# linomp/INF560-approximate-pattern-matching

Hardware: AMD Instinct MI355X
Metric: window-DP-cells/sec (higher is better)
Workload: dtype u32

## Files before the change

### inf560-approximate-pattern-matching_amd/csrc/apm_runtime.hip

```cpp
#include "apm_runtime.h"
#include "apm_core.h"

#include <cstdarg>
#include <cstdio>
#include <cstring>
#include <mutex>
#include <string>
#include <thread>
#include <vector>

static thread_local std::string g_create_error;

int fail(apm_ctx *ctx, int code, const char *fmt, ...) {
    char buf[512];
    va_list ap;
    va_start(ap, fmt);
    vsnprintf(buf, sizeof buf, fmt, ap);
    va_end(ap);
    static std::mutex mu;
    std::lock_guard<std::mutex> lock(mu);
    if (ctx) ctx->err = buf;
    else g_create_error = buf;
    return code;
}
// ... 236 lines not shown
            return fail(nullptr, APM_ERR_NO_DEVICE, "%d devices requested, APM_DEVICES lists %d", n_devices, (int)devs.size());
        return create_common(ctx, devs, true);
    }
    if (n_devices <= 0) n_devices = have;
    if (n_devices > have) return fail(nullptr, APM_ERR_NO_DEVICE, "%d devices requested, %d visible", n_devices, have);
    if (n_devices > apm_ctx::N_STAGE / 2) return fail(nullptr, APM_ERR_NO_DEVICE, "at most %d devices per context", apm_ctx::N_STAGE / 2);
    for (int i = 0; i < n_devices; ++i) devs.push_back(i);
    return create_common(ctx, devs, true);
}

int apm_create_on_device(apm_ctx **ctx, int device_id) {
    if (!ctx) return fail(nullptr, APM_ERR_INVALID, "ctx is NULL");
    *ctx = nullptr;
    const int have = apm_device_count();
    if (have < 0) return have;
    if (have == 0) return fail(nullptr, APM_ERR_NO_DEVICE, "no HIP device visible (this engine has no CPU fallback)");
    if (device_id < 0 || device_id >= have)
        return fail(nullptr, APM_ERR_NO_DEVICE, "device %d out of range (%d visible)", device_id, have);
    return create_common(ctx, std::vector<int>{device_id}, false);
}

void apm_destroy(apm_ctx *ctx) {
    if (!ctx) return;
    for (apm_ctx *ch : ctx->children) apm_destroy(ch);
    ctx->children.clear();
    if (ctx->rccl.ready)
        for (void *c : ctx->rccl.comms) if (c) ctx->rccl.CommDestroy(c);
    for (auto &ds : ctx->devs) {
        if (ds.dev < 0) continue;
        hipSetDevice(ds.dev);
        if (ds.own_stream) hipStreamSynchronize(ds.own_stream);
        free_device_plan(ds);
        for (void *p : {(void *)ds.d_scratch, (void *)ds.d_text, (void *)ds.d_rec, (void *)ds.d_rec_n, (void *)ds.d_ops, (void *)ds.d_masks, (void *)ds.d_stats,
                        (void *)ds.d_work, (void *)ds.d_blist, (void *)ds.d_clist, (void *)ds.d_clist_cnt, (void *)ds.d_raw, (void *)ds.d_tn_summary,
                        (void *)ds.d_tn_map, (void *)ds.d_tn_total, (void *)ds.d_sq_count, (void *)ds.d_sq_prefix, (void *)ds.d_sq_total,
                        (void *)ds.d_seq_table, (void *)ds.d_loc_buf, (void *)ds.d_best})
            if (p) hipFree(p);
        for (hipEvent_t e : ds.ev_best) if (e) hipEventDestroy(e);
        for (hipEvent_t e : ds.ev_stage) if (e) hipEventDestroy(e);
        for (hipEvent_t e : ds.ev_launch) if (e) hipEventDestroy(e);
        for (hipEvent_t e : ds.ev_tn) if (e) hipEventDestroy(e);
        for (hipEvent_t e : ds.ev_sq) if (e) hipEventDestroy(e);
        for (hipEvent_t e : {ds.ev_start, ds.ev_kstart, ds.ev_mstart, ds.ev_mstop, ds.ev_stop}) if (e) hipEventDestroy(e);
        if (ds.own_stream) hipStreamDestroy(ds.own_stream);
    }
    for (int b = 0; b < apm_ctx::N_STAGE; ++b)
        if (ctx->stage[b]) hipHostFree(ctx->stage[b]);
    delete ctx;
}

int apm_set_stream(apm_ctx *ctx, void *hip_stream) {
    if (!ctx) return APM_ERR_INVALID;
    if (ctx->devs.size() != 1) return fail(ctx, APM_ERR_STATE, "apm_set_stream needs a single-device context");
    ctx->devs[0].stream = hip_stream == APM_STREAM_OWN ? ctx->devs[0].own_stream : (hipStream_t)hip_stream;
    return APM_OK;
}

int apm_set_partition(apm_ctx *ctx, int partition) {
    if (!ctx) return APM_ERR_INVALID;
    if (partition != APM_PARTITION_TEXT && partition != APM_PARTITION_PATTERNS) return fail(ctx, APM_ERR_INVALID, "unknown partition %d", partition);
    if (partition == ctx->partition) return APM_OK;
    ctx->partition = partition;
    return ctx->pats.empty() ? (int)APM_OK : rebuild(ctx);
}

int apm_set_patterns(apm_ctx *ctx, int n_patterns, const char *const *pat, const int *len, int k) {
    if (!ctx) return APM_ERR_INVALID;
// ... 130 lines not shown
```

### inf560-approximate-pattern-matching_amd/csrc/apm_scan.hip

```cpp
#include "apm_state.h"
#include "apm_core.h"

#include <algorithm>
#include <cstdlib>
#include <cstring>

__global__ void apm_popcount_kernel(const uint32_t *w, unsigned long long n, unsigned long long *sum) {
    unsigned long long acc = 0;
    for (unsigned long long i = (unsigned long long)blockIdx.x * blockDim.x + threadIdx.x; i < n; i += (unsigned long long)gridDim.x * blockDim.x)
        acc += (unsigned long long)__popc(w[i]);
    for (int d = 32; d; d >>= 1) acc += __shfl_down(acc, d, 64);
    if ((threadIdx.x & 63) == 0 && acc) atomicAdd(sum, acc);
}

__global__ void apm_popcount_listed_kernel(const uint32_t *w, const uint32_t *blist, const uint32_t *n_listed, const uint32_t *clist_cnt, int regions, unsigned long long *sum) {
    unsigned long long acc = 0;
    const unsigned long long n = (unsigned long long)*n_listed * 64ull, t0 = (unsigned long long)blockIdx.x * blockDim.x + threadIdx.x;
    for (unsigned long long i = t0; i < n; i += (unsigned long long)gridDim.x * blockDim.x)
        acc += (unsigned long long)__popc(w[(unsigned long long)blist[i >> 6] * 64ull + (i & 63ull)]);
    for (unsigned long long i = t0; i < (unsigned long long)regions; i += (unsigned long long)gridDim.x * blockDim.x) acc += clist_cnt[i];
    for (int d = 32; d; d >>= 1) acc += __shfl_down(acc, d, 64);
    if ((threadIdx.x & 63) == 0 && acc) atomicAdd(sum, acc);
}

// ... 15 lines not shown
        const unsigned long long i = b0 + threadIdx.x, at = s_base + threadIdx.x;
        if (i < total && at < cap) {
            const unsigned long long pos = ob + i % span;
            out[at] = make_uint4((uint32_t)pos, (uint32_t)(pos >> 32), (uint32_t)idx[i / span], 0u);
        }
    }
}

int note_launch(apm_ctx *ctx, DeviceState &ds, const char *label) {
    ds.launches++;
    if (!ctx->timing_on || ds.n_stamps >= DeviceState::MAX_STAMPS) return APM_OK;
    hipEvent_t &e = ds.ev_launch[ds.n_stamps];
    if (!e) HIP_TRY(ctx, hipEventCreate(&e));
    HIP_TRY(ctx, hipEventRecord(e, ds.stream));
    ds.launch_label[ds.n_stamps++] = label;
    return APM_OK;
}

int ensure_text(apm_ctx *ctx, DeviceState &ds, size_t bytes) {
    bytes = (bytes + 255) & ~(size_t)255;
    if (bytes <= ds.text_cap) return APM_OK;
    HIP_TRY(ctx, hipSetDevice(ds.dev));
    return grow_device_buffer(ctx, ds, (void **)&ds.d_text, &ds.text_cap, bytes, 1);
}

static int env_int(const char *name, int unset) { const char *v = getenv(name); return v ? atoi(v) : unset; }
static int env_1_to_64(const char *name, int unset) { return getenv(name) ? std::max(1, std::min(64, env_int(name, 0))) : unset; }
struct ScanEnv {
    int fused = env_int("APM_FUSED", -1);
    int blist = env_int("APM_SIEVE_BLIST", 1);
    int clist = env_int("APM_SIEVE_CLIST", 1);
    int clist_region_cap = env_1_to_64("APM_CLIST_REGION_CAP", 0);
    int clist_min_batch = env_1_to_64("APM_CLIST_MIN_BATCH", 8);
    int cf_dp_diag = env_int("APM_CF_DP_DIAG", 1);
    int filter_dma = env_int("APM_FILTER_DMA", 1);
    int filter_stream = env_int("APM_FILTER_STREAM", 1);
#ifdef APM_MEASURE
    int qcap_s1 = env_int("APM_QCAP_S1", 0);
    int bpc_cap = env_int("APM_BPC_CAP", 0);
#endif
};
static const ScanEnv &scan_env() {
    static const ScanEnv env;
    return env;
}

struct ShardGeom {
    const uint8_t *text;
    int64_t jb, je;
    int64_t nrel;
    int64_t avail;
    int64_t avail_pad;
    int band;
    ApmPosSink sink;
    unsigned long long *counts;
    bool rec_on;
    bool aligned() const { return (reinterpret_cast<uintptr_t>(text) & 15u) == 0; }
};
#define APM_PICK(g, fn) ((g).rec_on ? fn##_rec : fn)

template <typename Args> static void set_common(Args &a, const apm_ctx *ctx, const ShardGeom &g, int64_t je) {
    a.text = g.text;
    a.jb = g.jb;
    a.je = je;
    a.nrel = g.nrel;
    a.counts = g.counts;
// ... 24 lines not shown
static int launch_generic_group(apm_ctx *ctx, DeviceState &ds, const ShardGeom &g, const GenericGroup &grp, const ApmPatDesc *d_descs, int mode) {
    if (grp.descs.empty() || g.je <= g.jb) return APM_OK;
    int64_t span = g.je - g.jb;
    if (mode == 1) span = std::min<int64_t>(span, grp.m_max);
    const size_t col = (size_t)grp.m_max + 1;
    const size_t budget = (size_t)1 << 30;
    const size_t per_launch = std::min<size_t>(grp.descs.size(), 65535);
    int64_t nbx = (span + APM_BLOCK - 1) / APM_BLOCK;
    const int64_t cap = std::max<int64_t>(1, (int64_t)(budget / (col * 2 * APM_BLOCK * per_launch)));
    nbx = std::max<int64_t>(1, std::min<int64_t>(std::min<int64_t>(nbx, cap), 4096));
    const size_t need = col * 2 * APM_BLOCK * (size_t)nbx * per_launch;
    const int rc = grow_device_buffer(ctx, ds, (void **)&ds.d_scratch, &ds.scratch_bytes, need, 1);
    if (rc) return rc;
    ApmGenericArgs a{};
    set_common(a, ctx, g, g.je);
    a.avail = g.avail;
    a.bytes = ds.d_allpat;
    a.mode = mode;
    a.col_stride = (int)col;
    a.scratch = ds.d_scratch;
    for (size_t first = 0; first < grp.descs.size(); first += per_launch) {
        a.pats = d_descs + first;
        APM_LAUNCH(ctx, ds, "generic", APM_PICK(g, apm_launch_generic)(a, (int)nbx, (int)std::min(per_launch, grp.descs.size() - first), ds.stream));
    }
    return APM_OK;
}

struct SieveRange {
    int64_t p_lo, p_hi;
    int64_t n_mask_blocks = 0;
    const uint32_t *blist_ctr = nullptr;
    int clist_regions = 0;
    uint32_t clist_region_cap = 0;
    int64_t nchunks() const { return (p_hi - p_lo + 1023) / 1024; }
};
constexpr int kClistPerBlock = 32;
constexpr int kClistMaxRegions = 4096;

static ApmSieve2Args sieve_args(const SievePlan &S, const ShardGeom &g, const SieveRange &r, const uint32_t *d_bitmap) {
    ApmSieve2Args sv{};
    sv.text = g.text;
    sv.avail_pad = g.avail_pad;
    sv.tile0 = r.p_lo;
    sv.nchunks = r.nchunks();
    sv.bitmap = reinterpret_cast<const uint4 *>(d_bitmap);
    sv.code_shift = S.code_shift;
    sv.stride = S.stride;
    return sv;
}

static ApmVerifyArgs verify_args(const apm_ctx *ctx, const VerifyLaunch &V, const DevVerify &D, const ShardGeom &g, int64_t je_v) {
    const SievePlan &S = ctx->plan.sieve;
    ApmVerifyArgs va{};
    set_common(va, ctx, g, je_v);
    va.avail = g.avail;
    va.avail_pad = g.avail_pad;
    va.image = reinterpret_cast<const uint4 *>(D.d_image);
    va.image_len = (int)V.image.size();
    va.o_prefix = V.o_prefix;
    va.o_r2s = V.o_r2s;
    va.o_slots = V.o_slots;
    va.o_kext = V.o_kext;
    va.o_pat = V.o_pat;
    va.o_masks = V.o_masks;
    va.o_kinfo = V.o_kinfo;
    va.o_pinfo = V.o_pinfo;
// ... 18 lines not shown
    for (size_t v = 0; fused_ok && v < S.launches.size(); ++v) {
        const VerifyLaunch &V = S.launches[v];
        DevVerify &D = ds.verify[v];
        ApmFusedArgs fa{};
        fa.s = sieve_args(S, g, r, ds.d_sieve_bmp);
        fa.v = verify_args(ctx, V, D, g, std::min<int64_t>(g.je, g.nrel - V.m_min + 1));
#ifdef APM_MEASURE
        if (!ds.d_stats) HIP_TRY(ctx, hipMalloc((void **)&ds.d_stats, APM_STATS_BYTES));
        fa.v.stats = ds.d_stats;
#endif
        if (!D.fused_threads) {
            D.fused_blocks_per_cu = apm_fused_geometry(fa, &D.fused_threads);
            if (D.fused_blocks_per_cu < 1) D.fused_threads = -1;
        }
        if (D.fused_threads < 64) fused_ok = false;
        if (fa.v.je > g.jb) { fargs.push_back(fa); fa_index.push_back(v); }
    }
    if (!fused_ok) return APM_OK;
    for (ApmFusedArgs &fa : fargs) {
        tails.ride_with(fa.s);
        const DevVerify &D = ds.verify[fa_index[&fa - fargs.data()]];
#ifdef APM_MEASURE
        HIP_TRY(ctx, hipMemsetAsync(ds.d_stats, 0, APM_STATS_BYTES, ds.stream));
#endif
        fa.v.work = ds.d_work;
        APM_LAUNCH(ctx, ds, "fused", APM_PICK(g, apm_launch_fused)(fa, D.fused_threads, ds.n_cu * D.fused_blocks_per_cu, &ds.work_epoch, ds.stream));
    }
    *ran = true;
    return APM_OK;
}

static int sieve_pass(apm_ctx *ctx, DeviceState &ds, const ShardGeom &g, SieveRange &r, ShortTails &tails, int v) {
    const SievePlan &S = ctx->plan.sieve;
    ApmSieve2Args sv = sieve_args(S, g, r, v < 0 ? ds.d_sieve_bmp : ds.verify[(size_t)v].d_bmp18);
    sv.masks = ds.d_masks;
    if (v >= 0) {
        const VerifyLaunch &V = S.launches[(size_t)v];
        const DevVerify &D = ds.verify[(size_t)v];
        sv.cf_image = reinterpret_cast<const uint4 *>(D.d_cf);
        sv.cf_len = (int)V.cf_image.size();
        sv.cf_o_rrec = V.cf_o_rrec;
        sv.cf_o_lrec = V.cf_o_lrec;
        sv.cf_threads = D.cf_threads;
        sv.cf_blocks_per_cu = D.cf_blocks_per_cu;
        sv.cf_o_dp = V.cf_o_dp;
        sv.cf_dp_k = ctx->k;
        sv.cf_dp_cols = V.cf_dp_cols;
    }
    if (v < 0 || tails.n <= 512) tails.ride_with(sv);
    const bool use_blist = scan_env().blist && sv.cf_image != nullptr;
    r.blist_ctr = nullptr;
    if (use_blist) {
        sv.blist = ds.d_blist;
        sv.blist_ctr = APM_BLIST_CTR(ds.d_work, ds.sieve_epoch & 1);
        sv.blist_ctr_next = APM_BLIST_CTR(ds.d_work, (ds.sieve_epoch + 1) & 1);
        r.blist_ctr = sv.blist_ctr;
    }
    r.clist_regions = 0;
    if (use_blist && scan_env().clist) {
        const size_t want = (size_t)r.n_mask_blocks * (size_t)kClistPerBlock + (size_t)kClistMaxRegions * 64;
        const int grc = grow_device_buffer(ctx, ds, (void **)&ds.d_clist, &ds.clist_cap, want, 4);
        if (grc) return grc;
        if (!ds.d_clist_cnt) HIP_TRY(ctx, hipMalloc((void **)&ds.d_clist_cnt, (size_t)kClistMaxRegions * 4));
        const int regions = apm_sieve2cf_blocks(sv, ds.n_cu);
        if (regions >= 1 && regions <= kClistMaxRegions) {
            r.clist_regions = regions;
            r.clist_region_cap = scan_env().clist_region_cap ? (uint32_t)scan_env().clist_region_cap
                                                             : (uint32_t)std::max<int64_t>(64, r.n_mask_blocks * kClistPerBlock / regions);
            sv.clist = ds.d_clist;
            sv.clist_cnt = ds.d_clist_cnt;
            sv.clist_cap = r.clist_region_cap;
        }
    }
    ds.last_clist_regions = r.clist_regions;
    ds.last_blist_ctr = r.blist_ctr;
    HIP_TRY(ctx, APM_PICK(g, apm_launch_sieve2)(sv, ds.n_cu, ds.stream, scan_env().cf_dp_diag != 0, &ds.last_sieve_waves, &ds.last_cf_dp_form));
    if (use_blist) ++ds.sieve_epoch;
    return note_launch(ctx, ds, "sieve");
}

static int verify_pass(apm_ctx *ctx, DeviceState &ds, const ShardGeom &g, const SieveRange &r, size_t v, int64_t je_v) {
    DevVerify &D = ds.verify[v];
    ApmVerifyArgs va = verify_args(ctx, ctx->plan.sieve.launches[v], D, g, je_v);
    va.masks = ds.d_masks;
    if (r.blist_ctr) {
        va.blist = ds.d_blist;
        va.blist_ctr = r.blist_ctr;
    }
    if (r.clist_regions) {
        va.clist = ds.d_clist;
        va.clist_cnt = ds.d_clist_cnt;
        va.clist_cap = r.clist_region_cap;
        va.clist_regions = r.clist_regions;
        va.clist_min_batch = scan_env().clist_min_batch;
    }
    va.tile0 = r.p_lo;
    va.n_mask_blocks = r.n_mask_blocks;
#ifdef APM_MEASURE
    if (!ds.d_stats) HIP_TRY(ctx, hipMalloc((void **)&ds.d_stats, APM_STATS_BYTES));
    HIP_TRY(ctx, hipMemsetAsync(ds.d_stats, 0, APM_STATS_BYTES, ds.stream));
    va.stats = ds.d_stats;
#endif
    va.work = ds.d_work;
    if (!D.blocks_per_cu) D.blocks_per_cu = apm_verify_geometry(va, &D.threads);
    APM_LAUNCH(ctx, ds, "verify", APM_PICK(g, apm_launch_verify)(va, D.threads, ds.n_cu * D.blocks_per_cu, &ds.work_epoch, ds.stream));
    return APM_OK;
}

static int run_sieve_verify(apm_ctx *ctx, DeviceState &ds, const ShardGeom &g, SieveRange &r, ShortTails &tails) {
    const SievePlan &S = ctx->plan.sieve;
    r.n_mask_blocks = (r.nchunks() + 3) / 4;
    int rc = grow_device_buffer(ctx, ds, (void **)&ds.d_masks, &ds.masks_cap, (size_t)r.n_mask_blocks * 64 + 64, 4);
    if (rc) return rc;
    rc = grow_device_buffer(ctx, ds, (void **)&ds.d_blist, &ds.blist_cap, (size_t)r.n_mask_blocks + 64, 4);
    if (rc) return rc;
    ds.last_mask_blocks = r.n_mask_blocks;
    bool per_launch = S.per_launch_sieve;
    for (size_t v = 0; per_launch && v < S.launches.size(); ++v) {
        const VerifyLaunch &V = S.launches[v];
        DevVerify &D = ds.verify[v];
        if (!D.cf_threads) {
            D.cf_blocks_per_cu = apm_sieve2cf_geometry((int)V.cf_image.size(), apm_cf_dp_form(V.cf_o_dp > 0, ctx->k, scan_env().cf_dp_diag != 0), &D.cf_threads);
// ... 209 lines not shown
    ShardGeom g{};
    g.text = d_text;
    g.jb = (int64_t)(ob - text_off);
    g.je = (int64_t)(oe - text_off);
    g.nrel = (int64_t)(n_total - text_off);
    g.avail = (int64_t)text_len;
    g.avail_pad = g.avail + (int64_t)((16u - ((reinterpret_cast<uintptr_t>(d_text) + (uintptr_t)g.avail) & 15u)) & 15u);
    g.band = ctx->k / 2;
    g.counts = d_counts;
    g.rec_on = rec != nullptr;
    if (rec) {
        g.sink = *rec;
        g.sink.text_off = text_off;
    } else if (ctx->find_active) {
        g.sink.out = ds.d_pos_out;
        g.sink.count = ds.d_pos_count;
        g.sink.cap = ds.pos_cap;
        g.sink.text_off = text_off;
    }
    ShortTails tails;
    set_common(tails.args, ctx, g, g.je);
    tails.args.pats = ds.d_stail_descs;
    tails.args.bytes = ds.d_allpat;
    tails.n = (int)plan.stails.descs.size();
    tails.pending = has_tail_windows(plan.stails, g);

    if (ctx->timing_on) HIP_TRY(ctx, hipEventRecord(ds.ev_mstart, ds.stream));
    bool fused_run = false, sieve_run = false;
    int rc = run_sieve_pipeline(ctx, ds, g, tails, &fused_run, &sieve_run);
    if (rc) return rc;
    rc = run_tiled_launches(ctx, ds, g, tails, fused_run || sieve_run);
    if (rc) return rc;
    ds.last_fused = fused_run;
    if (!sieve_run) { ds.last_mask_blocks = 0; ds.last_clist_regions = 0; ds.last_sieve_waves = 0; ds.last_cf_dp_form = 0; }
    rc = launch_generic_group(ctx, ds, g, plan.longs, ds.d_long_descs, 2);
    if (rc) return rc;
    if (ctx->timing_on) HIP_TRY(ctx, hipEventRecord(ds.ev_mstop, ds.stream));
    if (has_tail_windows(plan.tails, g)) {
        rc = launch_generic_group(ctx, ds, g, plan.tails, ds.d_tail_descs, 1);
        if (rc) return rc;
    }
    return run_tails_and_trivial(ctx, ds, g, tails, ob, oe);
}

int scan_shard(apm_ctx *ctx, DeviceState &ds, const ShardText &sh, uint64_t own_begin, uint64_t own_end, unsigned long long *d_counts,
               const ApmPosSink *rec) {
    const uint8_t *d_text = sh.text;
    uint64_t text_off = sh.text_off, text_len = sh.text_len;
    const uint64_t n_total = sh.n_total;
    const bool sieve_on = ctx->plan.sieve.on;
    const uint64_t lim32 = (uint64_t)APM_SIEVE_MAX_BYTES - 4096;
    const uint64_t mis = (uint64_t)(reinterpret_cast<uintptr_t>(d_text) & 15u);
    if (sieve_on && mis != 0 && text_off >= mis && text_len > 0) {
        d_text -= mis;
        text_off -= mis;
        text_len += mis;
    }
    if (!sieve_on || text_len < lim32 || (reinterpret_cast<uintptr_t>(d_text) & 15u) != 0 || own_begin < text_off)
        return scan_shard_one(ctx, ds, ShardText{d_text, text_off, text_len, n_total}, own_begin, own_end, d_counts, rec);
    const uint64_t k = (uint64_t)ctx->k;
    const uint64_t oe = std::min(own_end, n_total > k ? n_total - k : 0);
    const uint64_t m_max = (uint64_t)std::max(ctx->plan.m_max, 1), step = (uint64_t)3 << 30;
    for (uint64_t b = own_begin; b < oe;) {
        const uint64_t e = std::min(oe, b + step);
        const uint64_t sb = text_off + ((b - text_off) & ~(uint64_t)15);
        const uint64_t se = std::min(text_off + text_len, e + m_max + 31);
        const int rc = scan_shard_one(ctx, ds, ShardText{d_text + (sb - text_off), sb, se - sb, n_total}, b, e, d_counts, rec);
// ... 24 lines not shown
```

### inf560-approximate-pattern-matching_amd/csrc/apm_sieve.h

```cpp
#ifndef APM_SIEVE_H
#define APM_SIEVE_H

#include "apm_internal.h"

struct ApmSieve2Args {
    const uint8_t *text;
    int64_t avail_pad;
    int64_t tile0;
    int64_t nchunks;
    const uint4 *bitmap;
    int code_shift;
    int stride;
    uint32_t *masks;
    uint32_t *blist;
    uint32_t *blist_ctr, *blist_ctr_next;
    uint32_t *clist;
    uint32_t *clist_cnt;
    uint32_t clist_cap;
    int n_main_blocks;
    int n_tail;
    ApmTailArgs tail;
    const uint4 *cf_image;
    int cf_len, cf_o_rrec, cf_o_lrec;
    int cf_o_dp, cf_dp_k, cf_dp_cols;
    int cf_threads, cf_blocks_per_cu;
#ifdef APM_MEASURE
    int skip_mask;
#endif
};
#define APM_SIEVE_MAX_BYTES (((int64_t)1 << 32) - ((int64_t)64 << 20))
#define APM_CF_WAVE_BYTES 1552
#define APM_CF_DP_PEND_BYTES 128
#define APM_CF_DP_COLS 30
#define APM_CF_DP_SLOTS 7
static inline int apm_cf_dp_form(bool dp, int k, bool diag_on) { return !dp ? 0 : (diag_on && k <= 3 ? 2 : 1); }
const void *apm_sieve2cfdg_fn();
int apm_sieve2cf_geometry(int cf_len, int dp_form, int *threads);
int apm_sieve2cf_blocks(const ApmSieve2Args &a, int n_cu);

struct ApmVerifyArgs {
    const uint8_t *text;
    int64_t avail;
    int64_t avail_pad;
    int64_t jb, je, nrel;
    const uint4 *image;
    int image_len, o_prefix, o_r2s, o_slots, o_kext, o_pat;
    int o_masks;
    int o_rc;
    int o_kinfo, o_pinfo;
    const uint32_t *kinfo;
    const uint2 *pinfo;
    const uint32_t *kpart;
    const ApmPatDesc *pats;
    unsigned long long *counts;
    int n_pats, nk, k, band, code_shift;
    int stride;
    const uint32_t *masks;
    const uint32_t *blist;
    const uint32_t *blist_ctr;
    const uint32_t *clist;
    const uint32_t *clist_cnt;
    uint32_t clist_cap;
    int clist_regions;
    int clist_min_batch;
    int64_t tile0;
    int64_t n_mask_blocks;
    int n_blocks;
    uint32_t *work;
    int work_epoch;
    int work_groups;
#ifdef APM_MEASURE
    int skip_mask;
    unsigned long long *stats;
#endif
    ApmPosSink pos;
};

struct ApmFusedArgs {
    ApmSieve2Args s;
    ApmVerifyArgs v;
};
#define APM_FUSED_MAX_THREADS 896
hipError_t apm_launch_fused(const ApmFusedArgs &a, int threads, int max_blocks, int *work_epoch, hipStream_t s);
size_t apm_fused_lds_bytes(const ApmFusedArgs &a, int threads);
int apm_fused_geometry(const ApmFusedArgs &a, int *threads);

#define APM_WORK_GROUPS 32
#define APM_WORK_STRIDE 64
#define APM_WORK_BYTES (2 * APM_WORK_GROUPS * APM_WORK_STRIDE * 4 + 2 * APM_WORK_STRIDE * 4)
#define APM_BLIST_CTR(work, set) ((work) + 2 * APM_WORK_GROUPS * APM_WORK_STRIDE + (set) * APM_WORK_STRIDE)
#define APM_STATS_WAVES 16384
#define APM_STATS_BYTES (64 + 16 * APM_STATS_WAVES)
hipError_t apm_launch_sieve2(const ApmSieve2Args &a, int n_cu, hipStream_t s, bool dp_diag, int *cf_waves, int *cf_dp_form);
hipError_t apm_launch_verify(const ApmVerifyArgs &a, int threads, int max_blocks, int *work_epoch, hipStream_t s);
int apm_verify_geometry(const ApmVerifyArgs &a, int *threads);
#ifndef APM_REC
hipError_t apm_launch_fused_rec(const ApmFusedArgs &a, int threads, int max_blocks, int *work_epoch, hipStream_t s);
hipError_t apm_launch_sieve2_rec(const ApmSieve2Args &a, int n_cu, hipStream_t s, bool dp_diag, int *cf_waves, int *cf_dp_form);
hipError_t apm_launch_verify_rec(const ApmVerifyArgs &a, int threads, int max_blocks, int *work_epoch, hipStream_t s);
#endif

#endif
```

### inf560-approximate-pattern-matching_amd/csrc/apm_sieve.hip

```cpp
#include "apm_wave.h"
#include "apm_sieve.h"
#include "apm_launch.h"
#include "apm_sieve_body.h"


__global__ __launch_bounds__(APM_SIEVE2_BLOCK, 8) void apm_sieve2_kernel(ApmSieve2Args a) {
    extern __shared__ __attribute__((aligned(16))) uint8_t smem[];
    apm_sieve2_body<false, false>(a, smem);
}

__global__ __launch_bounds__(1024, 8) void apm_sieve2cf_kernel(ApmSieve2Args a) {
    extern __shared__ __attribute__((aligned(16))) uint8_t smem[];
    apm_sieve2_body<true, false>(a, smem);
}
__global__ __launch_bounds__(1024, 8) void apm_sieve2cfdp_kernel(ApmSieve2Args a) {
    extern __shared__ __attribute__((aligned(16))) uint8_t smem[];
    apm_sieve2_body<true, true>(a, smem);
}

__global__ __launch_bounds__(APM_SIEVE2_BLOCK, 8) void apm_sieve8_kernel(ApmSieve2Args a) {
    extern __shared__ __attribute__((aligned(16))) uint8_t smem[];
    const int tid = threadIdx.x, lane = tid & 63;
    const int wv = __builtin_amdgcn_readfirstlane(tid >> 6);
    if ((int)blockIdx.x >= a.n_main_blocks) {
// ... 33 lines not shown
        { const u32x4 v = r2; load_chunk(c + 4 * W + 2, r2); h2 = hit_bits(v, c + 2); }
        { const u32x4 v = r3; load_chunk(c + 4 * W + 3, r3); h3 = hit_bits(v, c + 3); }
        a.masks[(size_t)(c >> 2) * 64 + (size_t)lane] = h0 | (h1 << 8) | (h2 << 16) | (h3 << 24);
    }
}

static size_t apm_sieve2cf_lds_bytes(int cf_len, int threads, bool dp) {
    return (size_t)32768 + (size_t)cf_len + (size_t)(threads / 64) * (APM_CF_WAVE_BYTES + (dp ? APM_CF_DP_PEND_BYTES : 0)) + 16;
}

static const void *apm_sieve2cf_fn(int dp_form) {
    return dp_form == 2 ? apm_sieve2cfdg_fn() : dp_form == 1 ? (const void *)apm_sieve2cfdp_kernel : (const void *)apm_sieve2cf_kernel;
}

int apm_sieve2cf_geometry(int cf_len, int dp_form, int *threads) {
    const bool dp = dp_form != 0;
    const void *fn = apm_sieve2cf_fn(dp_form);
    apm_ensure_max_lds(fn);
#ifdef APM_MEASURE
    static const int forced = getenv("APM_CF_THREADS") ? atoi(getenv("APM_CF_THREADS")) : 0;
#else
    constexpr int forced = 0;
#endif
    return apm_best_geometry([&](int) { return fn; }, 1024, 256, -64, [&](int t) { return apm_sieve2cf_lds_bytes(cf_len, t, dp); }, INT_MAX, forced, threads);
}

int apm_sieve2cf_blocks(const ApmSieve2Args &a, int n_cu) {
    const int wpb = a.cf_threads / 64;
    if (a.nchunks <= 0 || wpb < 1 || a.cf_blocks_per_cu < 1) return 0;
    const int64_t want = (a.nchunks + 4 * wpb - 1) / (4 * wpb), cap = (int64_t)n_cu * a.cf_blocks_per_cu;
    return (int)(want < cap ? want : cap);
}

hipError_t apm_launch_sieve2(const ApmSieve2Args &a, int n_cu, hipStream_t s, bool dp_diag, int *cf_waves, int *cf_dp_form) {
    if (cf_waves) *cf_waves = 0;
    if (cf_dp_form) *cf_dp_form = 0;
    if (a.nchunks <= 0) return hipSuccess;
    if (a.avail_pad > APM_SIEVE_MAX_BYTES || a.tile0 < 0) return hipErrorInvalidValue;
    ApmSieve2Args args = a;
#ifdef APM_MEASURE
    if (const char *e = getenv("APM_MEASURE_SKIP")) args.skip_mask = atoi(e);
#endif
    void *kargs[] = {&args};
    if (a.stride != 8 && a.cf_image) {
        const int threads = a.cf_threads;
        if (threads < 128 || threads > 1024 || (threads & 63) || a.cf_blocks_per_cu < 1) return hipErrorInvalidValue;
        const int64_t nb = apm_sieve2cf_blocks(a, n_cu);
        if (a.clist && (!a.blist || !a.clist_cnt || a.clist_cap < 1u)) return hipErrorInvalidValue;
        args.n_main_blocks = (int)nb;
#ifdef APM_CF_NODP
        const bool dp = false;
#else
        const bool dp = a.clist && a.cf_o_dp > 0;
#endif
        if (dp && (a.cf_dp_cols < 1 || a.cf_dp_cols > APM_CF_DP_COLS || a.cf_dp_k < 0 || a.cf_o_dp + 128 > a.cf_len)) return hipErrorInvalidValue;
        const int dp_form = apm_cf_dp_form(dp, a.cf_dp_k, dp_diag);
        const void *fn = apm_sieve2cf_fn(dp_form);
        const size_t lds = apm_sieve2cf_lds_bytes(a.cf_len, threads, dp);
        if (lds > (size_t)160 * 1024) return hipErrorInvalidValue;
        if (lds > 48 * 1024) apm_ensure_max_lds(fn);
        if (cf_dp_form) *cf_dp_form = dp_form;
        if (cf_waves) *cf_waves = (int)nb * (threads / 64);
        return hipLaunchKernel(fn, dim3((unsigned)(nb + a.n_tail)), dim3((unsigned)threads), kargs, lds, s);
    }
    const size_t lds = 32768;
    const int64_t want = (a.nchunks + 4 * (APM_SIEVE2_BLOCK / 64) - 1) / (4 * (APM_SIEVE2_BLOCK / 64));
    const int64_t cap = (int64_t)n_cu * 4;
    const int64_t nb = want < cap ? want : cap;
    args.n_main_blocks = (int)nb;
    if (a.stride == 8)
        return hipLaunchKernel((const void *)apm_sieve8_kernel, dim3((unsigned)(nb + a.n_tail)), dim3(APM_SIEVE2_BLOCK), kargs, 8192, s);
    return hipLaunchKernel((const void *)apm_sieve2_kernel, dim3((unsigned)(nb + a.n_tail)), dim3(APM_SIEVE2_BLOCK), kargs, lds, s);
}
```

### inf560-approximate-pattern-matching_amd/csrc/apm_sieve_body.h

```cpp
#ifndef APM_SIEVE_BODY_H
#define APM_SIEVE_BODY_H
#include "apm_wave.h"
#include "apm_sieve.h"

#define APM_SIEVE2_BLOCK 512

template <bool CF, bool DP, bool DIAG = false>
__device__ __forceinline__ void apm_sieve2_body(const ApmSieve2Args &a, uint8_t *smem) {
    const int THREADS = CF ? (int)blockDim.x : APM_SIEVE2_BLOCK;
    constexpr uint32_t WAVE_BYTES = APM_CF_WAVE_BYTES + (DP ? APM_CF_DP_PEND_BYTES : 0);
    const int tid = threadIdx.x, lane = tid & 63;
    const int wv = __builtin_amdgcn_readfirstlane(tid >> 6);
    if ((int)blockIdx.x >= a.n_main_blocks) {
        apm_tail_body(a.tail, (int)blockIdx.x - a.n_main_blocks, reinterpret_cast<uint4 *>(smem), tid);
        return;
    }
    apm_stage_image(reinterpret_cast<uint4 *>(smem), a.bitmap, 2048, tid, THREADS);
    if constexpr (CF) apm_stage_image(reinterpret_cast<uint4 *>(smem + 32768), a.cf_image, a.cf_len >> 4, tid, THREADS);
    uint32_t *cl_ctr = reinterpret_cast<uint32_t *>(smem + 32768 + (CF ? a.cf_len + (THREADS / 64) * WAVE_BYTES : 0));
    if (CF && tid == 0) { cl_ctr[0] = 0u; cl_ctr[1] = DP ? 0u : 0xffffffffu; }
    __syncthreads();
    const int64_t W = (int64_t)a.n_main_blocks * (THREADS / 64);
    const int64_t nch = a.nchunks;

    const __amdgpu_buffer_rsrc_t rs_all =
        __builtin_amdgcn_make_buffer_rsrc(const_cast<uint8_t *>(a.text), 0, (int)(uint32_t)a.avail_pad, 0x00020000);
    const uint32_t t0_32 = (uint32_t)a.tile0, lane16 = 16u * (uint32_t)lane;
    auto load_chunk = [&](int64_t cc, u32x4 &r) __attribute__((always_inline)) {
        r = __builtin_amdgcn_raw_buffer_load_b128(rs_all, (int)(t0_32 + (uint32_t)cc * 1024u + lane16), 0, 0);
    };
    auto load_tail = [&](int64_t cc, v2u32 &tl) __attribute__((always_inline)) {
        tl = __builtin_amdgcn_raw_buffer_load_b64(rs_all, (int)(t0_32 + (uint32_t)cc * 1024u), 0, 0);
    };
    auto load_halo = [&](int64_t cc, u32x4 &hl) __attribute__((always_inline)) {
        const uint32_t g = (uint32_t)(a.tile0 + cc * 1024);
        const uint32_t off = lane < 2 ? g + 4096u + 16u * (uint32_t)lane : (lane == 2 ? g - 16u : 0xfffffff0u);
        hl = __builtin_amdgcn_raw_buffer_load_b128(rs_all, (int)off, 0, 0);
    };
    const uint32_t cs = (uint32_t)a.code_shift;
    auto pack16 = [&](const u32x4 &v) __attribute__((always_inline)) { return apm_pack16(v.x, v.y, v.z, v.w, cs); };
    auto hit_bits = [&](uint32_t slo, uint32_t nx0, int64_t cc) __attribute__((always_inline)) {
        uint32_t hits = apm_lookup2_chunk(slo, nx0);
#ifdef APM_MEASURE
// ... 249 lines not shown
                    }
                    const uint32_t t = has ? (uint32_t)__builtin_ctz(hm) : 0u;
                    hm &= hm - 1u;
                    if (has)
                        region[base + apm_wave_rank(mask)] = e0 + 512u * (t >> 3) + (t & 7u);
                }
            }
            const bool any = __builtin_amdgcn_ballot_w64(hm != 0u) != 0ull;
            if (!a.clist || any) a.masks[(size_t)(c >> 2) * 64 + (size_t)lane] = hm;
            if (a.blist && any) {
                if ((uint32_t)lane == bl_n) bl_pend = (uint32_t)(c >> 2);
                if (++bl_n == 64u) bl_flush();
            }
        } else {
            a.masks[(size_t)(c >> 2) * 64 + (size_t)lane] = hm;
        }
    }
    if (DP && qn) dp_flush();
    if constexpr (CF) {
        if (a.blist) {
            if ((uint32_t)lane < bl_n) st[lane] = bl_pend;
            if (lane == 0) st[64] = bl_n;
            __syncthreads();
            uint32_t *wg = reinterpret_cast<uint32_t *>(smem + 32768 + a.cf_len);
            const uint32_t nw = (uint32_t)(THREADS / 64);
            uint32_t before = 0, total = 0;
            for (uint32_t w = 0; w < nw; ++w) {
                const uint32_t cw = wg[w * (WAVE_BYTES / 4) + 64];
                if (w < (uint32_t)wv) before += cw;
                total += cw;
            }
            uint32_t *gbase = wg + 65;
            if (tid == 0 && total) *gbase = __hip_atomic_fetch_add(a.blist_ctr, total, __ATOMIC_RELAXED, __HIP_MEMORY_SCOPE_AGENT);
            __syncthreads();
            if ((uint32_t)lane < bl_n) a.blist[*gbase + before + (uint32_t)lane] = bl_pend;
            if (a.clist && tid == 0) a.clist_cnt[blockIdx.x] = DP ? cl_ctr[0] : (cl_ctr[0] < cl_ctr[1] ? cl_ctr[0] : cl_ctr[1]);
        }
    }
}

#endif
```

### inf560-approximate-pattern-matching_amd/csrc/apm_sieve_diag.hip

```cpp
#include "apm_sieve_body.h"

__global__ __launch_bounds__(1024, 8) void apm_sieve2cfdg_kernel(ApmSieve2Args a) {
    extern __shared__ __attribute__((aligned(16))) uint8_t smem[];
    apm_sieve2_body<true, true, true>(a, smem);
}

const void *apm_sieve2cfdg_fn() { return (const void *)apm_sieve2cfdg_kernel; }
```

### inf560-approximate-pattern-matching_amd/csrc/apm_state.h

```cpp
#ifndef APM_STATE_H
#define APM_STATE_H

#include "../../include/apm.h"
#include "apm_plan.h"
#include "apm_sieve.h"
#include "apm_textnorm.h"
#include "apm_seqindex.h"

#include <string>
#include <vector>

struct DevVerify {
    uint32_t *d_bmp18 = nullptr;
    uint8_t *d_cf = nullptr;
    ApmPatDesc *d_descs = nullptr;
    uint8_t *d_image = nullptr;
    uint32_t *d_kinfo = nullptr;
    uint32_t *d_pinfo = nullptr;
    uint32_t *d_kpart = nullptr;
    int blocks_per_cu = 0, threads = 256;
    int fused_blocks_per_cu = 0, fused_threads = 0;
    int cf_threads = 0, cf_blocks_per_cu = 0;
};

// ... 53 lines not shown
    bool tn_valid = false;
    uint64_t tn_src_bytes = 0, tn_kept_bytes = 0;
    hipEvent_t ev_tn[4] = {};
    bool tn_timed = false, map_timed = false;
    uint32_t *d_sq_count = nullptr;
    unsigned long long *d_sq_prefix = nullptr;
    unsigned long long *d_sq_total = nullptr;
    size_t sq_cap = 0;
    uint64_t sq_n_seq = 0;
    bool tn_host = false;
    apm_seq *d_seq_table = nullptr;
    size_t seq_table_cap = 0;
    uint64_t seq_table_n = 0;
    uint8_t *d_loc_buf = nullptr;
    size_t loc_buf_cap = 0;
    hipEvent_t ev_sq[4] = {};
    bool sq_timed = false, locate_timed = false;
    hipEvent_t ev_stage[32] = {};
    uint32_t *d_sieve_bmp = nullptr;
    std::vector<DevVerify> verify;
    uint32_t *d_masks = nullptr;
    size_t masks_cap = 0;
    int64_t last_mask_blocks = 0;
    uint32_t *d_work = nullptr;
    int work_epoch = 0;
    uint32_t *d_blist = nullptr;
    size_t blist_cap = 0;
    int sieve_epoch = 0;
    uint32_t *d_clist = nullptr;
    uint32_t *d_clist_cnt = nullptr;
    size_t clist_cap = 0;
    int last_clist_regions = 0;
    const uint32_t *last_blist_ctr = nullptr;
    unsigned long long *d_stats = nullptr;
    int last_sieve_waves = 0;
    int last_cf_dp_form = 0;
    bool last_fused = false;
    hipEvent_t ev_start = nullptr, ev_kstart = nullptr, ev_mstart = nullptr, ev_mstop = nullptr, ev_stop = nullptr;
    bool events_recorded = false;
    static constexpr int MAX_STAMPS = 32;
    hipEvent_t ev_launch[MAX_STAMPS] = {};
    const char *launch_label[MAX_STAMPS] = {};
    int n_stamps = 0;
    uint64_t text_bytes = 0;
    int launches = 0;
};

struct RcclApi {
    void *handle = nullptr;
    int (*CommInitAll)(void **, int, const int *) = nullptr;
    int (*CommDestroy)(void *) = nullptr;
    int (*AllReduce)(const void *, void *, size_t, int, int, void *, hipStream_t) = nullptr;
    int (*GroupStart)() = nullptr;
    int (*GroupEnd)() = nullptr;
    std::vector<void *> comms;
    bool ready = false;
};

struct apm_ctx {
    std::vector<DeviceState> devs;
    std::vector<PatternInfo> pats;
    ApmPlan plan;
    int k = 0;
    int kernel = APM_KERNEL_AUTO;
    bool patterns_set = false;
    bool timing_on = true;
// ... 48 lines not shown
```

### inf560-approximate-pattern-matching_amd/csrc/apm_stats.hip

```cpp
#include "apm_runtime.h"
#include "apm_core.h"

#include <cstdlib>
#include <string>
#include <vector>

void account(apm_ctx *ctx, uint64_t n_total, uint64_t ob, uint64_t oe) {
    const uint64_t k = (uint64_t)ctx->k;
    const uint64_t limit = n_total > k ? n_total - k : 0;
    oe = std::min(oe, limit);
    if (oe <= ob) return;
    for (const auto &p : ctx->pats) {
        const uint64_t m = (uint64_t)p.m;
        const uint64_t full_end = n_total >= m ? std::min<uint64_t>(oe, n_total - m + 1) : 0;
        const uint64_t nfull = full_end > ob ? full_end - ob : 0;
        double cells = double(nfull) * double(m) * double(m);
        for (uint64_t j = std::max(ob, full_end); j < oe; ++j) {
            const double s = double(n_total - j);
            cells += s * s;
        }
        ctx->timing.windows += oe - ob;
        ctx->timing.cells_algorithmic += cells;
        if (p.kernel == APM_KERNEL_BANDED || p.kernel == APM_KERNEL_NFA)
            ctx->timing.cells_evaluated += double(oe - ob) * double(m) * double(2 * (ctx->k / 2) + 1);
// ... 58 lines not shown
    DeviceState &ds = ctx->devs[0];
    if (!ds.events_recorded || ds.n_stamps == 0) return 0;
    HIP_TRY(ctx, hipSetDevice(ds.dev));
    HIP_TRY(ctx, hipEventSynchronize(ds.ev_launch[ds.n_stamps - 1]));
    const int n = std::min(max, ds.n_stamps);
    for (int i = 0; i < n; ++i) {
        float t = 0;
        if (hipEventElapsedTime(&t, i ? ds.ev_launch[i - 1] : ds.ev_mstart, ds.ev_launch[i]) != hipSuccess) t = 0;
        ms[i] = t;
        if (labels) labels[i] = ds.launch_label[i];
    }
    return n;
}

int apm_get_stat(const apm_ctx *cctx, const char *name, double *value) {
    apm_ctx *ctx = const_cast<apm_ctx *>(cctx);
    if (!ctx || !name || !value || ctx->devs.empty()) return APM_ERR_INVALID;
    DeviceState &ds = ctx->devs[0];
    const std::string n = name;
    const SievePlan &S = ctx->plan.sieve;
    static const DevVerify no_verify;
    const DevVerify &G0 = ds.verify.empty() ? no_verify : ds.verify[0];
    if (n == "sieve_on") { *value = S.on ? 1 : 0; return APM_OK; }
    if (n == "sieve_rate") { *value = S.rate; return APM_OK; }
    if (n == "sieve_fused") { *value = ds.last_fused ? 1 : 0; return APM_OK; }
    if (n == "sieve_cf") { *value = (S.on && S.per_launch_sieve && G0.cf_threads >= 64) ? (double)G0.cf_threads : 0.0; return APM_OK; }
    if (n == "sieve_weak_frac") { *value = S.weak_frac; return APM_OK; }
    if (n == "sieve_cf_dp_slots") { *value = S.per_launch_sieve ? (double)S.launches[0].cf_dp_slots : 0.0; return APM_OK; }
    if (n == "sieve_cf_dp_form") { *value = (double)ds.last_cf_dp_form; return APM_OK; }
    if (n == "sieve_cf_waves_per_cu") { *value = (S.per_launch_sieve && G0.cf_threads >= 64) ? (double)(G0.cf_threads / 64 * G0.cf_blocks_per_cu) : 0.0; return APM_OK; }
    if (n == "sieve_cf_bytes") { *value = S.per_launch_sieve ? (double)S.launches[0].cf_image.size() : 0.0; return APM_OK; }
    if (n == "sieve_stride") { *value = S.on ? (double)S.stride : 0.0; return APM_OK; }
    if (n == "sieve_clist") { *value = ds.last_clist_regions ? 1.0 : 0.0; return APM_OK; }
    if (n == "sieve_waves") { *value = (double)ds.last_sieve_waves; return APM_OK; }
    if (n == "sieve_mask_bytes") {
        *value = (double)ds.last_mask_blocks * 256.0;
        if (ds.last_clist_regions && ds.last_mask_blocks > 0) {
            HIP_TRY(ctx, hipSetDevice(ds.dev));
            std::vector<uint32_t> cnt((size_t)ds.last_clist_regions);
            uint32_t listed = 0;
            HIP_TRY(ctx, hipMemcpyAsync(cnt.data(), ds.d_clist_cnt, cnt.size() * 4, hipMemcpyDeviceToHost, ds.stream));
            HIP_TRY(ctx, hipMemcpyAsync(&listed, ds.last_blist_ctr, 4, hipMemcpyDeviceToHost, ds.stream));
            HIP_TRY(ctx, hipStreamSynchronize(ds.stream));
            double entries = 0;
            for (uint32_t c : cnt) entries += (double)c;
            *value = 4.0 * entries + 256.0 * (double)listed;
        }
        return APM_OK;
    }
    if (n == "verify_launches") { *value = (double)S.launches.size(); return APM_OK; }
    if (n == "verify_image_bytes") { *value = S.launches.empty() ? 0.0 : (double)S.launches[0].image.size(); return APM_OK; }
    if (n == "verify_blocks_per_cu") {
        *value = S.launches.empty() ? 0.0 : (double)(ds.last_fused ? G0.fused_blocks_per_cu : G0.blocks_per_cu);
        return APM_OK;
    }
    if (n == "verify_threads") {
        *value = S.launches.empty() ? 0.0 : (double)(ds.last_fused ? G0.fused_threads : G0.threads);
        return APM_OK;
    }
    if (n == "sieve_candidates") return sieve_candidates(ctx, ds, value);
    if (n == "align_rows") { *value = (double)ds.last_align_rows; return APM_OK; }
    if (n == "norm_src_bytes") { *value = (double)ds.tn_src_bytes; return APM_OK; }
    if (n == "norm_kept_bytes") { *value = (double)ds.tn_kept_bytes; return APM_OK; }
    if (n == "seq_count") { *value = (double)ds.sq_n_seq; return APM_OK; }
    if (n == "seq_index_ms" || n == "locate_ms") {
        const int at = n == "seq_index_ms" ? 0 : 2;
// ... 93 lines not shown
```

Baseline: 785200000 billion.

## Compact per-region candidate lists into a few shared pools for verify

The diagonal DP sieve kernel now copies each block's candidate list into one of a small number of shared pools (eight by default) using an atomic offset. The pool counters are double-buffered by epoch so block 0 can zero the next epoch's counters without a separate memset. Verify then reads a few dense pools instead of thousands of sparse per-region lists, which is meant to cut per-region scanning overhead and load imbalance in verify. In exchange the sieve does extra global atomics and copies, and uses more device memory.

```diff
diff --git a/inf560-approximate-pattern-matching_amd/csrc/apm_runtime.hip b/inf560-approximate-pattern-matching_amd/csrc/apm_runtime.hip
--- a/inf560-approximate-pattern-matching_amd/csrc/apm_runtime.hip
+++ b/inf560-approximate-pattern-matching_amd/csrc/apm_runtime.hip
@@ -292,7 +292,7 @@
         if (ds.own_stream) hipStreamSynchronize(ds.own_stream);
         free_device_plan(ds);
         for (void *p : {(void *)ds.d_scratch, (void *)ds.d_text, (void *)ds.d_rec, (void *)ds.d_rec_n, (void *)ds.d_ops, (void *)ds.d_masks, (void *)ds.d_stats,
-                        (void *)ds.d_work, (void *)ds.d_blist, (void *)ds.d_clist, (void *)ds.d_clist_cnt, (void *)ds.d_raw, (void *)ds.d_tn_summary,
+                        (void *)ds.d_work, (void *)ds.d_blist, (void *)ds.d_clist, (void *)ds.d_clist_cnt, (void *)ds.d_cpool, (void *)ds.d_cpool_cnt, (void *)ds.d_raw, (void *)ds.d_tn_summary,
                         (void *)ds.d_tn_map, (void *)ds.d_tn_total, (void *)ds.d_sq_count, (void *)ds.d_sq_prefix, (void *)ds.d_sq_total,
                         (void *)ds.d_seq_table, (void *)ds.d_loc_buf, (void *)ds.d_best})
             if (p) hipFree(p);
diff --git a/inf560-approximate-pattern-matching_amd/csrc/apm_scan.hip b/inf560-approximate-pattern-matching_amd/csrc/apm_scan.hip
--- a/inf560-approximate-pattern-matching_amd/csrc/apm_scan.hip
+++ b/inf560-approximate-pattern-matching_amd/csrc/apm_scan.hip
@@ -71,6 +71,7 @@
     int clist = env_int("APM_SIEVE_CLIST", 1);
     int clist_region_cap = env_1_to_64("APM_CLIST_REGION_CAP", 0);
     int clist_min_batch = env_1_to_64("APM_CLIST_MIN_BATCH", 8);
+    int clist_pools = std::max(0, env_int("APM_CLIST_POOLS", 8));
     int cf_dp_diag = env_int("APM_CF_DP_DIAG", 1);
     int filter_dma = env_int("APM_FILTER_DMA", 1);
     int filter_stream = env_int("APM_FILTER_STREAM", 1);
@@ -161,6 +162,9 @@
     const uint32_t *blist_ctr = nullptr;
     int clist_regions = 0;
     uint32_t clist_region_cap = 0;
+    int clist_pools = 0;
+    uint32_t clist_pool_cap = 0;
+    const uint32_t *cpool_cnt = nullptr;
     int64_t nchunks() const { return (p_hi - p_lo + 1023) / 1024; }
 };
 constexpr int kClistPerBlock = 32;
@@ -245,7 +249,8 @@
 
 static int sieve_pass(apm_ctx *ctx, DeviceState &ds, const ShardGeom &g, SieveRange &r, ShortTails &tails, int v) {
     const SievePlan &S = ctx->plan.sieve;
-    ApmSieve2Args sv = sieve_args(S, g, r, v < 0 ? ds.d_sieve_bmp : ds.verify[(size_t)v].d_bmp18);
+    ApmSieve2PoolArgs sv{};
+    static_cast<ApmSieve2Args &>(sv) = sieve_args(S, g, r, v < 0 ? ds.d_sieve_bmp : ds.verify[(size_t)v].d_bmp18);
     sv.masks = ds.d_masks;
     if (v >= 0) {
         const VerifyLaunch &V = S.launches[(size_t)v];
@@ -285,10 +290,35 @@
             sv.clist_cap = r.clist_region_cap;
         }
     }
+    r.clist_pools = 0;
+    if (r.clist_regions && scan_env().clist_pools > 0 && apm_cf_dp_form(sv.cf_o_dp > 0, sv.cf_dp_k, scan_env().cf_dp_diag != 0) == 2) {
+        const int pools = std::min(scan_env().clist_pools, r.clist_regions);
+        r.clist_pool_cap = (uint32_t)((r.clist_regions + pools - 1) / pools) * r.clist_region_cap;
+        const int grc = grow_device_buffer(ctx, ds, (void **)&ds.d_cpool, &ds.cpool_cap, (size_t)pools * r.clist_pool_cap, 4);
+        if (grc) return grc;
+        if (!ds.d_cpool_cnt) {
+            HIP_TRY(ctx, hipMalloc((void **)&ds.d_cpool_cnt, (size_t)2 * kClistMaxRegions * 4));
+            HIP_TRY(ctx, hipMemsetAsync(ds.d_cpool_cnt, 0, (size_t)2 * kClistMaxRegions * 4, ds.stream));
+        }
+        sv.cpool = ds.d_cpool;
+        sv.cpool_cnt = ds.d_cpool_cnt + (size_t)(ds.pool_epoch & 1) * kClistMaxRegions;
+        sv.cpool_cnt_next = ds.d_cpool_cnt + (size_t)((ds.pool_epoch + 1) & 1) * kClistMaxRegions;
+        sv.cpool_cap = r.clist_pool_cap;
+        sv.cpool_n = pools;
+        sv.cpool_next_n = ds.pool_dirty[(ds.pool_epoch + 1) & 1];
+        r.cpool_cnt = sv.cpool_cnt;
+    }
     ds.last_clist_regions = r.clist_regions;
     ds.last_blist_ctr = r.blist_ctr;
-    HIP_TRY(ctx, APM_PICK(g, apm_launch_sieve2)(sv, ds.n_cu, ds.stream, scan_env().cf_dp_diag != 0, &ds.last_sieve_waves, &ds.last_cf_dp_form));
+    ds.last_clist_pools = 0;
+    HIP_TRY(ctx, APM_PICK(g, apm_launch_sieve2)(sv, ds.n_cu, ds.stream, scan_env().cf_dp_diag != 0, &ds.last_sieve_waves, &ds.last_cf_dp_form, &r.clist_pools));
+    ds.last_clist_pools = r.clist_pools;
     if (use_blist) ++ds.sieve_epoch;
+    if (r.clist_pools) {
+        ds.pool_dirty[ds.pool_epoch & 1] = r.clist_pools;
+        ds.pool_dirty[(ds.pool_epoch + 1) & 1] = 0;
+        ++ds.pool_epoch;
+    }
     return note_launch(ctx, ds, "sieve");
 }
 
@@ -300,7 +330,13 @@
         va.blist = ds.d_blist;
         va.blist_ctr = r.blist_ctr;
     }
-    if (r.clist_regions) {
+    if (r.clist_pools) {
+        va.clist = ds.d_cpool;
+        va.clist_cnt = r.cpool_cnt;
+        va.clist_cap = r.clist_pool_cap;
+        va.clist_regions = r.clist_pools;
+        va.clist_min_batch = scan_env().clist_min_batch;
+    } else if (r.clist_regions) {
         va.clist = ds.d_clist;
         va.clist_cnt = ds.d_clist_cnt;
         va.clist_cap = r.clist_region_cap;
@@ -576,7 +612,7 @@
     rc = run_tiled_launches(ctx, ds, g, tails, fused_run || sieve_run);
     if (rc) return rc;
     ds.last_fused = fused_run;
-    if (!sieve_run) { ds.last_mask_blocks = 0; ds.last_clist_regions = 0; ds.last_sieve_waves = 0; ds.last_cf_dp_form = 0; }
+    if (!sieve_run) { ds.last_mask_blocks = 0; ds.last_clist_regions = 0; ds.last_clist_pools = 0; ds.last_sieve_waves = 0; ds.last_cf_dp_form = 0; }
     rc = launch_generic_group(ctx, ds, g, plan.longs, ds.d_long_descs, 2);
     if (rc) return rc;
     if (ctx->timing_on) HIP_TRY(ctx, hipEventRecord(ds.ev_mstop, ds.stream));
diff --git a/inf560-approximate-pattern-matching_amd/csrc/apm_sieve.h b/inf560-approximate-pattern-matching_amd/csrc/apm_sieve.h
--- a/inf560-approximate-pattern-matching_amd/csrc/apm_sieve.h
+++ b/inf560-approximate-pattern-matching_amd/csrc/apm_sieve.h
@@ -27,6 +27,13 @@
 #ifdef APM_MEASURE
     int skip_mask;
 #endif
+};
+struct ApmSieve2PoolArgs : ApmSieve2Args {
+    uint32_t *cpool;
+    uint32_t *cpool_cnt, *cpool_cnt_next;
+    uint32_t cpool_cap;
+    int cpool_n;
+    int cpool_next_n;
 };
 #define APM_SIEVE_MAX_BYTES (((int64_t)1 << 32) - ((int64_t)64 << 20))
 #define APM_CF_WAVE_BYTES 1552
@@ -91,12 +98,12 @@
 #define APM_BLIST_CTR(work, set) ((work) + 2 * APM_WORK_GROUPS * APM_WORK_STRIDE + (set) * APM_WORK_STRIDE)
 #define APM_STATS_WAVES 16384
 #define APM_STATS_BYTES (64 + 16 * APM_STATS_WAVES)
-hipError_t apm_launch_sieve2(const ApmSieve2Args &a, int n_cu, hipStream_t s, bool dp_diag, int *cf_waves, int *cf_dp_form);
+hipError_t apm_launch_sieve2(const ApmSieve2PoolArgs &a, int n_cu, hipStream_t s, bool dp_diag, int *cf_waves, int *cf_dp_form, int *clist_pools);
 hipError_t apm_launch_verify(const ApmVerifyArgs &a, int threads, int max_blocks, int *work_epoch, hipStream_t s);
 int apm_verify_geometry(const ApmVerifyArgs &a, int *threads);
 #ifndef APM_REC
 hipError_t apm_launch_fused_rec(const ApmFusedArgs &a, int threads, int max_blocks, int *work_epoch, hipStream_t s);
-hipError_t apm_launch_sieve2_rec(const ApmSieve2Args &a, int n_cu, hipStream_t s, bool dp_diag, int *cf_waves, int *cf_dp_form);
+hipError_t apm_launch_sieve2_rec(const ApmSieve2PoolArgs &a, int n_cu, hipStream_t s, bool dp_diag, int *cf_waves, int *cf_dp_form, int *clist_pools);
 hipError_t apm_launch_verify_rec(const ApmVerifyArgs &a, int threads, int max_blocks, int *work_epoch, hipStream_t s);
 #endif
 
diff --git a/inf560-approximate-pattern-matching_amd/csrc/apm_sieve.hip b/inf560-approximate-pattern-matching_amd/csrc/apm_sieve.hip
--- a/inf560-approximate-pattern-matching_amd/csrc/apm_sieve.hip
+++ b/inf560-approximate-pattern-matching_amd/csrc/apm_sieve.hip
@@ -89,12 +89,13 @@
     return (int)(want < cap ? want : cap);
 }
 
-hipError_t apm_launch_sieve2(const ApmSieve2Args &a, int n_cu, hipStream_t s, bool dp_diag, int *cf_waves, int *cf_dp_form) {
+hipError_t apm_launch_sieve2(const ApmSieve2PoolArgs &a, int n_cu, hipStream_t s, bool dp_diag, int *cf_waves, int *cf_dp_form, int *clist_pools) {
     if (cf_waves) *cf_waves = 0;
     if (cf_dp_form) *cf_dp_form = 0;
+    if (clist_pools) *clist_pools = 0;
     if (a.nchunks <= 0) return hipSuccess;
     if (a.avail_pad > APM_SIEVE_MAX_BYTES || a.tile0 < 0) return hipErrorInvalidValue;
-    ApmSieve2Args args = a;
+    ApmSieve2PoolArgs args = a;
 #ifdef APM_MEASURE
     if (const char *e = getenv("APM_MEASURE_SKIP")) args.skip_mask = atoi(e);
 #endif
@@ -113,10 +114,20 @@
         if (dp && (a.cf_dp_cols < 1 || a.cf_dp_cols > APM_CF_DP_COLS || a.cf_dp_k < 0 || a.cf_o_dp + 128 > a.cf_len)) return hipErrorInvalidValue;
         const int dp_form = apm_cf_dp_form(dp, a.cf_dp_k, dp_diag);
         const void *fn = apm_sieve2cf_fn(dp_form);
+        const bool pooled = dp_form == 2 && a.cpool != nullptr;
+        if (pooled) {
+            if (!a.cpool_cnt || !a.cpool_cnt_next || a.cpool_n < 1 || a.cpool_next_n < 0) return hipErrorInvalidValue;
+            args.cpool_n = (int)std::min<int64_t>(a.cpool_n, nb);
+            const int64_t regions_per_pool = (nb + args.cpool_n - 1) / args.cpool_n;
+            if ((int64_t)a.cpool_cap < regions_per_pool * (int64_t)a.clist_cap) return hipErrorInvalidValue;
+        } else {
+            args.cpool = nullptr;
+        }
         const size_t lds = apm_sieve2cf_lds_bytes(a.cf_len, threads, dp);
         if (lds > (size_t)160 * 1024) return hipErrorInvalidValue;
         if (lds > 48 * 1024) apm_ensure_max_lds(fn);
         if (cf_dp_form) *cf_dp_form = dp_form;
+        if (clist_pools) *clist_pools = pooled ? args.cpool_n : 0;
         if (cf_waves) *cf_waves = (int)nb * (threads / 64);
         return hipLaunchKernel(fn, dim3((unsigned)(nb + a.n_tail)), dim3((unsigned)threads), kargs, lds, s);
     }
diff --git a/inf560-approximate-pattern-matching_amd/csrc/apm_sieve_body.h b/inf560-approximate-pattern-matching_amd/csrc/apm_sieve_body.h
--- a/inf560-approximate-pattern-matching_amd/csrc/apm_sieve_body.h
+++ b/inf560-approximate-pattern-matching_amd/csrc/apm_sieve_body.h
@@ -1,14 +1,17 @@
 #ifndef APM_SIEVE_BODY_H
 #define APM_SIEVE_BODY_H
+#include <type_traits>
 #include "apm_wave.h"
 #include "apm_sieve.h"
 
 #define APM_SIEVE2_BLOCK 512
 
-template <bool CF, bool DP, bool DIAG = false>
-__device__ __forceinline__ void apm_sieve2_body(const ApmSieve2Args &a, uint8_t *smem) {
+template <bool CF, bool DP, bool DIAG = false, typename Args = ApmSieve2Args>
+__device__ __forceinline__ void apm_sieve2_body(const Args &a, uint8_t *smem) {
     const int THREADS = CF ? (int)blockDim.x : APM_SIEVE2_BLOCK;
-    constexpr uint32_t WAVE_BYTES = APM_CF_WAVE_BYTES + (DP ? APM_CF_DP_PEND_BYTES : 0);
+    constexpr bool POOL = std::is_same<Args, ApmSieve2PoolArgs>::value;
+    static_assert(!POOL || (DIAG && DP), "the pooled hand-over belongs to the diagonal kernel");
+    constexpr uint32_t WAVE_BYTES =APM_CF_WAVE_BYTES + (DP ? APM_CF_DP_PEND_BYTES : 0);
     const int tid = threadIdx.x, lane = tid & 63;
     const int wv = __builtin_amdgcn_readfirstlane(tid >> 6);
     if ((int)blockIdx.x >= a.n_main_blocks) {
@@ -324,9 +327,26 @@
             }
             uint32_t *gbase = wg + 65;
             if (tid == 0 && total) *gbase = __hip_atomic_fetch_add(a.blist_ctr, total, __ATOMIC_RELAXED, __HIP_MEMORY_SCOPE_AGENT);
+            if constexpr (POOL) {
+                if (a.cpool && tid == 0) {
+                    const uint32_t n = cl_ctr[0];
+                    if (n) wg[66] = __hip_atomic_fetch_add(&a.cpool_cnt[blockIdx.x % (uint32_t)a.cpool_n], n, __ATOMIC_RELAXED, __HIP_MEMORY_SCOPE_AGENT);
+                }
+            }
             __syncthreads();
             if ((uint32_t)lane < bl_n) a.blist[*gbase + before + (uint32_t)lane] = bl_pend;
             if (a.clist && tid == 0) a.clist_cnt[blockIdx.x] = DP ? cl_ctr[0] : (cl_ctr[0] < cl_ctr[1] ? cl_ctr[0] : cl_ctr[1]);
+            if constexpr (POOL) {
+                if (a.cpool) {
+                    const uint32_t n = cl_ctr[0] < a.clist_cap ? cl_ctr[0] : a.clist_cap;
+                    const uint32_t *region = a.clist + (size_t)blockIdx.x * a.clist_cap;
+                    uint32_t *pool = a.cpool + (size_t)(blockIdx.x % (uint32_t)a.cpool_n) * a.cpool_cap + (n ? wg[66] : 0u);
+                    for (uint32_t i = (uint32_t)tid; i < n; i += (uint32_t)THREADS)
+                        pool[i] = __hip_atomic_load(&region[i], __ATOMIC_RELAXED, __HIP_MEMORY_SCOPE_AGENT);
+                    if (blockIdx.x == 0)
+                        for (int i = tid; i < a.cpool_next_n; i += THREADS) a.cpool_cnt_next[i] = 0u;
+                }
+            }
         }
     }
 }
diff --git a/inf560-approximate-pattern-matching_amd/csrc/apm_sieve_diag.hip b/inf560-approximate-pattern-matching_amd/csrc/apm_sieve_diag.hip
--- a/inf560-approximate-pattern-matching_amd/csrc/apm_sieve_diag.hip
+++ b/inf560-approximate-pattern-matching_amd/csrc/apm_sieve_diag.hip
@@ -1,8 +1,8 @@
 #include "apm_sieve_body.h"
 
-__global__ __launch_bounds__(1024, 8) void apm_sieve2cfdg_kernel(ApmSieve2Args a) {
+__global__ __launch_bounds__(1024, 8) void apm_sieve2cfdg_kernel(ApmSieve2PoolArgs a) {
     extern __shared__ __attribute__((aligned(16))) uint8_t smem[];
-    apm_sieve2_body<true, true, true>(a, smem);
+    apm_sieve2_body<true, true, true, ApmSieve2PoolArgs>(a, smem);
 }
 
 const void *apm_sieve2cfdg_fn() { return (const void *)apm_sieve2cfdg_kernel; }
diff --git a/inf560-approximate-pattern-matching_amd/csrc/apm_state.h b/inf560-approximate-pattern-matching_amd/csrc/apm_state.h
--- a/inf560-approximate-pattern-matching_amd/csrc/apm_state.h
+++ b/inf560-approximate-pattern-matching_amd/csrc/apm_state.h
@@ -109,6 +109,12 @@
     size_t clist_cap = 0;
     int last_clist_regions = 0;
     const uint32_t *last_blist_ctr = nullptr;
+    uint32_t *d_cpool = nullptr;
+    uint32_t *d_cpool_cnt = nullptr;
+    size_t cpool_cap = 0;
+    int pool_epoch = 0;
+    int pool_dirty[2] = {0, 0};
+    int last_clist_pools = 0;
     unsigned long long *d_stats = nullptr;
     int last_sieve_waves = 0;
     int last_cf_dp_form = 0;
diff --git a/inf560-approximate-pattern-matching_amd/csrc/apm_stats.hip b/inf560-approximate-pattern-matching_amd/csrc/apm_stats.hip
--- a/inf560-approximate-pattern-matching_amd/csrc/apm_stats.hip
+++ b/inf560-approximate-pattern-matching_amd/csrc/apm_stats.hip
@@ -114,6 +114,7 @@
     if (n == "sieve_cf_bytes") { *value = S.per_launch_sieve ? (double)S.launches[0].cf_image.size() : 0.0; return APM_OK; }
     if (n == "sieve_stride") { *value = S.on ? (double)S.stride : 0.0; return APM_OK; }
     if (n == "sieve_clist") { *value = ds.last_clist_regions ? 1.0 : 0.0; return APM_OK; }
+    if (n == "sieve_clist_pools") { *value = (double)ds.last_clist_pools; return APM_OK; }
     if (n == "sieve_waves") { *value = (double)ds.last_sieve_waves; return APM_OK; }
     if (n == "sieve_mask_bytes") {
         *value = (double)ds.last_mask_blocks * 256.0;
```

New measurement: 801000000 billion (median of 6 runs). 1.02x the previous value.
